# anzeA/Tarok

Measured on AMD Instinct MI355X. Metric: env steps/sec at 65 536 parallel 4-player games; 1/2/4/8 MI355X, higher is better.
Workload: dtype u64

## Files before the change

### tarok_amd/csrc/tarok_env.hip

```cpp
#include "tarok_device.h"

#include <hip/hip_runtime.h>
#include <stdint.h>
#include <stdio.h>
#include <stdlib.h>
#include <string.h>
#include <type_traits>
#include <utility>

#include "../../include/tarok_env.h"

#define TK_BLOCK 256
#define TK_PF_SLOTS (4 * TK_BLOCK)
#define TK_GRAPH_CACHE 16
#define TK_REFILL_CAP (TK_BLOCK * TK_AHEAD)
#define TK_REFILL_FAN 8
#define TK_RC(group, k) ((((size_t)(group)) * 4 + (k)) * 32)
#define TK_BULK_EVERY 32u
#define TK_BULK_CAP ((TK_BULK_EVERY / 4) * TK_BLOCK)

#define TK_AHEAD TAROK_GAMES_AHEAD
#define TK_LINE(episode) ((u32)(episode) % (u32)TK_AHEAD)
#define TK_FINQ 128
#define TK_STREAM_STORE(ptr, val) __builtin_nontemporal_store((val), (ptr))
// ... 53 lines not shown
#define HIPCHK(x)                                                   \
    do {                                                            \
        hipError_t e_ = (x);                                        \
        if (e_ != hipSuccess) { g_last_hip = (int)e_; return TAROK_EHIP; } \
    } while (0)

static inline dim3 grid_for(int64_t n) { return dim3((unsigned)((n + TK_BLOCK - 1) / TK_BLOCK)); }

__device__ __forceinline__ void load_game(Game &g, const ulonglong2 *s01, const ulonglong2 *s23, int64_t i) {
    ulonglong2 a = s01[i], b = s23[i];
    unpack(g, a.x, a.y, b.x, b.y);
}
__device__ __forceinline__ void store_game(const Game &g, ulonglong2 *s01, ulonglong2 *s23, int64_t i,
                                           bool seats_changed = true) {
    ulonglong2 a;
    pack_play(g, a.x, a.y);
    s01[i] = a;
    if (seats_changed) {
        ulonglong2 b;
        pack_seats(g, b.x, b.y);
        s23[i] = b;
    }
}

TK_KERNEL(TK_BLOCK, 80) void k_reset(
    int64_t n, u64 seed, u64 offset, u32 episode, int mix, int flags,
    const uint8_t *__restrict__ deals, const int8_t *__restrict__ contract, const int8_t *__restrict__ declarer,
    const int8_t *__restrict__ king, const int8_t *__restrict__ choice, const uint8_t *__restrict__ discards,
    ulonglong2 *__restrict__ s01, ulonglong2 *__restrict__ s23, Aux *aux, Counters *__restrict__ cnt,
    uint16_t *__restrict__ nstale, u64 *__restrict__ gkey) {
    TK_VGPR_TOP(80, 79);
    int64_t i = (int64_t)blockIdx.x * TK_BLOCK + threadIdx.x;
    if (i >= n) return;
    u64 key = game_key(seed, offset + (u64)i, episode);
    u64 h0 = 0, h1 = 0, h2 = 0, h3 = 0, tal = 0;
    bool bad = false;
#pragma unroll
    for (int b = 0; b < TK_AHEAD; b++) aux[i].line[b].nep = 0xFFFFFFFFu;
    nstale[i] = (uint16_t)((1u << TK_AHEAD) - 1);
    if (deals) {
        const uint8_t *p = deals + i * 54;
        u64 h[4] = {0, 0, 0, 0};
        u64 seen = 0;
        for (int k = 0; k < 48; k++) { u32 c = p[k]; bad |= c >= 54; c &= 63; seen |= 1ULL << c; h[k / 12] |= 1ULL << c; }
        for (int k = 0; k < 6; k++) { u32 c = p[48 + k]; bad |= c >= 54; c &= 63; seen |= 1ULL << c; tal |= (u64)c << (6 * k); }
        bad |= seen != TK_DECK;
        h0 = h[0]; h1 = h[1]; h2 = h[2]; h3 = h[3];
    } else {
        deal_thread(key, h0, h1, h2, h3, tal);
    }
    u32 c, d, k;
    if (contract) {
        int ci = contract[i];
        bad |= ci < 0 || ci > 9;
        c = (u32)ci % 10u;
        d = declarer ? ((u32)declarer[i] & 3u) : 0u;
        k = king ? ((u32)king[i] & 3u) : 0u;
    } else {
        sample_setup(key, mix, c, d, k);
    }
    Game g;
    setup_game(g, h0, h1, h2, h3, tal, c, d, k);
    g.epar = TK_LINE(episode); g.cprev = 0;
    if (g.phase == TK_PHASE_EXCHANGE && !(flags & TAROK_DEFER_EXCHANGE)) {
        if (choice && discards) {
            const uint8_t *q = discards + i * 3;
            apply_exchange(g, (u32)(uint8_t)choice[i], q[0], q[1], q[2]);
        } else {
            bot_exchange(g, key);
        }
    }
    if (bad) g.error = 1;
    store_game(g, s01, s23, i);
    gkey[i] = key;
    cnt[i].episode = episode;
    if (flags & TAROK_CLEAR_COUNTERS) cnt[i].score_sum = make_int4(0, 0, 0, 0);
}

__device__ __forceinline__ void deal_into_buffer(Aux *aux, int64_t j, u32 episode, u64 seed, u64 offset, int mix) {
    u64 key = game_key(seed, offset + (u64)j, (u64)episode);
    u64 h0, h1, h2, h3, tal;
    deal_thread(key, h0, h1, h2, h3, tal);
    u32 c, d, k;
    sample_setup(key, mix, c, d, k);
    Game g;
    setup_game(g, h0, h1, h2, h3, tal, c, d, k);
    g.epar = TK_LINE(episode); g.cprev = 0;
    if (g.phase == TK_PHASE_EXCHANGE) bot_exchange(g, key);
    ulonglong2 a, b;
    pack(g, a.x, a.y, b.x, b.y);
    AuxLine *ln = &aux[j].line[TK_LINE(episode)];
    ln->n01 = a; ln->n23 = b; ln->nkey = key; ln->nep = episode;
}

TK_KERNEL(TK_BLOCK, 128) void k_prefetch(int64_t n, u64 seed, u64 offset, int mix,
                                                      Aux *aux, const Counters *__restrict__ cnt,
                                                      uint16_t *__restrict__ nstale) {
    TK_VGPR_TOP(128, 127);
    __shared__ unsigned short list[TK_AHEAD * TK_PF_SLOTS];
    __shared__ u32 count;
    int64_t base = (int64_t)blockIdx.x * TK_PF_SLOTS;
    if (threadIdx.x == 0) count = 0;
    __syncthreads();
    const u64 ALL = (1u << TK_AHEAD) - 1;
    u64 f = reinterpret_cast<const u64 *>(nstale + base)[threadIdx.x];
    if (f) {
        u32 c = (u32)__popcll(f & (0x0001000100010001ULL * ALL));
        u32 pos = atomicAdd(&count, c);
#pragma unroll
        for (u32 k = 0; k < 4; k++) {
            u32 fk = (u32)(f >> (16 * k)) & (u32)ALL;
#pragma unroll
            for (u32 b = 0; b < TK_AHEAD; b++)
                if (fk & (1u << b)) list[pos++] = (unsigned short)((threadIdx.x * 4 + k) * TK_AHEAD + b);
        }
        reinterpret_cast<u64 *>(nstale + base)[threadIdx.x] = 0;
    }
    __syncthreads();
    u32 total = count;
    for (u32 j = threadIdx.x; j < total; j += TK_BLOCK) {
        int64_t i = base + list[j] / TK_AHEAD;
        if (i >= n) continue;
        deal_into_buffer(aux, i, cnt[i].episode + 1 + (list[j] % TK_AHEAD), seed, offset, mix);
    }
}

TK_KERNEL(TK_BLOCK, 64) void k_exchange(int64_t n, const int8_t *__restrict__ choice,
                                                      const uint8_t *__restrict__ discards,
                                                      ulonglong2 *__restrict__ s01, ulonglong2 *__restrict__ s23,
                                                      const u64 *__restrict__ gkey) {
    TK_VGPR_TOP(64, 63);
    int64_t i = (int64_t)blockIdx.x * TK_BLOCK + threadIdx.x;
    if (i >= n) return;
    Game g;
    load_game(g, s01, s23, i);
    if (g.phase != TK_PHASE_EXCHANGE) return;
    if (choice && discards) {
        const uint8_t *q = discards + i * 3;
        apply_exchange(g, (u32)(uint8_t)choice[i], q[0], q[1], q[2]);
    } else {
        bot_exchange(g, gkey[i]);
    }
    store_game(g, s01, s23, i);
}

TK_KERNEL(TK_BLOCK, 64) void k_legal(int64_t n, const ulonglong2 *__restrict__ s01,
                                                   const ulonglong2 *__restrict__ s23, u64 *__restrict__ obs,
                                                   int8_t *__restrict__ seat) {
    TK_VGPR_TOP(64, 63);
    int64_t i = (int64_t)blockIdx.x * TK_BLOCK + threadIdx.x;
    if (i >= n) return;
    Game g;
    load_game(g, s01, s23, i);
    obs[i] = obs_word(g, false);
    if (seat) seat[i] = (int8_t)((g.leader + g.nt) & 3);
}

TK_KERNEL(TK_BLOCK, 64) void k_policy(int64_t n, const u64 *__restrict__ obs,
                                                    const u64 *__restrict__ gkey, uint8_t *__restrict__ action) {
    TK_VGPR_TOP(64, 63);
    int64_t i = (int64_t)blockIdx.x * TK_BLOCK + threadIdx.x;
    if (i >= n) return;
    u64 o = obs[i], key = gkey[i];
    u64 m = o & TAROK_OBS_MASK;
    u32 a = 255;
    if (m) a = policy_action(key, (u32)(o >> TAROK_OBS_STEP_SHIFT) & 63u, m);
    action[i] = (uint8_t)a;
}

TK_KERNEL(TK_BLOCK, 64) void k_policy_x4(int64_t n, const u64 *__restrict__ obs,
                                                       const u64 *__restrict__ gkey, uint8_t *__restrict__ action) {
    TK_VGPR_TOP(64, 63);
    int64_t base = (int64_t)blockIdx.x * (4 * TK_BLOCK);
    if (base + 4 * TK_BLOCK <= n) {
        int64_t p0 = base + 2 * threadIdx.x, p1 = p0 + 2 * TK_BLOCK;
        ulonglong2 o0 = *reinterpret_cast<const ulonglong2 *>(obs + p0), o1 = *reinterpret_cast<const ulonglong2 *>(obs + p1);
        ulonglong2 k0 = *reinterpret_cast<const ulonglong2 *>(gkey + p0), k1 = *reinterpret_cast<const ulonglong2 *>(gkey + p1);
        auto one = [](u64 o, u64 key) __attribute__((always_inline)) {
            u64 m = o & TAROK_OBS_MASK;
            return m ? policy_action(key, (u32)(o >> TAROK_OBS_STEP_SHIFT) & 63u, m) : 255u;
        };
        u32 a0 = one(o0.x, k0.x) | (one(o0.y, k0.y) << 8), a1 = one(o1.x, k1.x) | (one(o1.y, k1.y) << 8);
        *reinterpret_cast<uint16_t *>(action + p0) = (uint16_t)a0;
        *reinterpret_cast<uint16_t *>(action + p1) = (uint16_t)a1;
        return;
    }
    for (int64_t i = base + threadIdx.x; i < n; i += TK_BLOCK) {
        u64 o = obs[i];
        u64 m = o & TAROK_OBS_MASK;
        u32 a = 255;
        if (m) a = policy_action(gkey[i], (u32)(o >> TAROK_OBS_STEP_SHIFT) & 63u, m);
        action[i] = (uint8_t)a;
    }
}

template <class T> __device__ __forceinline__ T tk_ld(const T *p) { return __hip_atomic_load(p, __ATOMIC_RELAXED, __HIP_MEMORY_SCOPE_AGENT); }

#define TK_EPOCH_SHARDS 256
#define TK_EPOCH_WORDS (32 * TK_EPOCH_SHARDS)
#define TK_PHASES (2u * TK_BULK_EVERY)
static_assert((TK_BULK_EVERY & (TK_BULK_EVERY - 1)) == 0 && TK_BULK_EVERY >= 4 && TK_BULK_EVERY + 1 <= 4 * (TK_AHEAD - 1),
              "a line is dealt at most TK_BULK_EVERY + 1 launches after it was emptied and is needed again TK_AHEAD - 1 games (four launches each, at least) after that");
struct TkCount { u32 own, other; };
__device__ __forceinline__ u32 tk_shard_size(u32 grid, u32 shard) { return (grid + TK_EPOCH_SHARDS - 1 - shard) / TK_EPOCH_SHARDS; }
template <int KIND> __device__ __forceinline__ u32 tk_other_grid(u32 groups, u32 fan) { return KIND == 0 ? groups + (groups + fan - 1) / fan : groups; }
template <int KIND> __device__ __forceinline__ u32 tk_other_shard(u32 groups) { return (KIND == 0 ? blockIdx.x : blockIdx.x % groups) % TK_EPOCH_SHARDS; }
template <int KIND> __device__ __forceinline__ TkCount launch_count(const u32 *epoch, u32 groups) {
    TkCount c;
    c.own = tk_ld(epoch + KIND * TK_EPOCH_WORDS + 32 * (blockIdx.x % TK_EPOCH_SHARDS));
    c.other = tk_ld(epoch + (1 - KIND) * TK_EPOCH_WORDS + 32 * tk_other_shard<KIND>(groups));
    return c;
}
__device__ __forceinline__ u32 tk_div_small(u32 count, u32 g) {
    u32 q = (u32)(((float)count + 0.5f) * __builtin_amdgcn_rcpf((float)g));
    q -= (q * g > count) ? 1u : 0u;
    q += ((q + 1u) * g <= count) ? 1u : 0u;
    return q;
}
template <int KIND> __device__ __forceinline__ u32 launch_phase(TkCount c, u32 groups, u32 fan) {
    asm volatile("" : "+v"(c.own), "+v"(c.other));
    u32 own = tk_div_small(c.own, tk_shard_size(gridDim.x, blockIdx.x % TK_EPOCH_SHARDS));
    u32 other = tk_div_small(c.other, tk_shard_size(tk_other_grid<KIND>(groups, fan), tk_other_shard<KIND>(groups)));
    return (own + other) % TK_PHASES;
}
template <int KIND> __device__ __forceinline__ void launch_counted(u32 *epoch) {
    if (threadIdx.x == 0)
        (void)atomicInc(epoch + KIND * TK_EPOCH_WORDS + 32 * (blockIdx.x % TK_EPOCH_SHARDS),
                        TK_PHASES * tk_shard_size(gridDim.x, blockIdx.x % TK_EPOCH_SHARDS) - 1u);
}

template <bool BULK>
__device__ __forceinline__ void refill_role(u32 rblock, u32 tid, u32 nthreads, u64 seed, u64 offset, int mix, u32 play_groups,
                                        TkCount count, u32 *epoch, u32 fan, bool bulk_on, Aux *aux, u64 *rlist, u32 *rcount, u64 *elist) {
    constexpr int KIND = BULK ? 0 : 1;
    const u32 kind_fan = fan;
    if (BULK) fan = 1;
    u32 g0 = rblock * fan;
    u32 len0[TK_REFILL_FAN], len1[TK_REFILL_FAN];
#pragma unroll
    for (u32 q = 0; q < TK_REFILL_FAN; q++) {
        bool has = q < fan && g0 + q < play_groups;
        len0[q] = has ? tk_ld(&rcount[TK_RC(g0 + q, 0)]) : 0u;
        len1[q] = has ? tk_ld(&rcount[TK_RC(g0 + q, 1)]) : 0u;
    }
    if (!BULK) {
        __syncthreads();
        launch_counted<KIND>(epoch);
    }
    const u32 phase = launch_phase<KIND>(count, play_groups, kind_fan), par = phase & 1u;
    if (!BULK) {
        if (tid < 2 * fan && g0 + tid / 2 < play_groups) rcount[TK_RC(g0 + tid / 2, 2 + (tid & 1))] = 0u;
    }
    u32 cum[TK_REFILL_FAN + 1];
    cum[0] = 0;
    u32 which = par ^ 1u;
    const u32 odd = 0u - par;
#pragma unroll
    for (u32 q = 0; q < TK_REFILL_FAN; q++) cum[q + 1] = cum[q] + ((len0[q] & odd) | (len1[q] & ~odd));
    const bool any = cum[TK_REFILL_FAN] != 0;
    u64 *lists = rlist;
    u32 cap = TK_REFILL_CAP;
    const bool bulk = BULK && bulk_on && phase % TK_BULK_EVERY == 0;
#pragma nounroll
    for (u32 pass = 0; pass < (BULK ? 2u : 1u); pass++) {
        if (pass == 1) {
            if (!bulk) break;
            which = ((phase / TK_BULK_EVERY) & 1u) ^ 1u;
            lists = elist; cap = TK_BULK_CAP;
#pragma unroll
            for (u32 q = 0; q < TK_REFILL_FAN; q++) {
                bool has = q < fan && g0 + q < play_groups;
                cum[q + 1] = cum[q] + (has ? min(tk_ld(&rcount[TK_RC(g0 + q, 2 + which)]), (u32)TK_BULK_CAP) : 0u);
            }
        }
        for (u32 j = tid; j < cum[TK_REFILL_FAN]; j += nthreads) {
            u32 q = 0;
#pragma unroll
            for (u32 r = 1; r < TK_REFILL_FAN; r++) q += j >= cum[r] ? 1u : 0u;
            u32 base = 0;
#pragma unroll
            for (u32 r = 0; r < TK_REFILL_FAN; r++) base = (r == q) ? cum[r] : base;
            u64 en = tk_ld(&lists[((int64_t)(g0 + q) * 2 + which) * cap + (j - base)]);
            deal_into_buffer(aux, (int64_t)(g0 + q) * TK_BLOCK + (u32)(en & 0xFFFF), (u32)(en >> 32), seed, offset, mix);
        }
    }
    if (any || bulk) {
        __syncthreads();
        if (any && tid < fan && g0 + tid < play_groups) rcount[TK_RC(g0 + tid, par ^ 1u)] = 0u;
        if (bulk && tid < fan && g0 + tid < play_groups) rcount[TK_RC(g0 + tid, 2 + which)] = 0u;
    }
}

template <bool HIST>
__device__ __forceinline__ void play_role(
    u32 group, u32 tid,
    int64_t n, u64 seed, u64 offset, int mix, int flags, int cards, int64_t stride, TkCount count, u32 *epoch, u32 play_groups, u32 fan,
    uint8_t *__restrict__ action_out, int16_t *__restrict__ reward,
    uint8_t *__restrict__ done, uint16_t *__restrict__ trick, u64 *__restrict__ obs, uint8_t *__restrict__ hist,
    ulonglong2 *__restrict__ s01, ulonglong2 *__restrict__ s23, Aux *aux, Counters *__restrict__ cnt,
    u64 *__restrict__ gkey, u64 *rlist, u32 *rcount, u64 *__restrict__ stamps) {
    __shared__ unsigned short push_list[TK_REFILL_CAP];
    __shared__ u32 push_ep[TK_BLOCK];
    __shared__ u32 push_count;
    __shared__ u32 finq[TK_BLOCK / 64][9][TK_FINQ];
    __shared__ int sacc[4][TK_BLOCK];
    if (tid == 0) push_count = 0;
    sacc[0][tid] = 0; sacc[1][tid] = 0; sacc[2][tid] = 0; sacc[3][tid] = 0;
    __syncthreads();
    u32 fq_head = 0, fq_n = 0;
    u32 (*fq)[TK_FINQ] = finq[tid >> 6];
    auto drain_finished = [&](u32 cnt_) __attribute__((always_inline)) {
        u32 lane = tid & 63;
        if (lane < cnt_) {
            u32 e = (fq_head + lane) & (TK_FINQ - 1);
            Game f;
            f.A = TK_U64(fq[0][e], fq[1][e]); f.B = TK_U64(fq[2][e], fq[3][e]); f.C = TK_U64(fq[4][e], fq[5][e]);
            u32 m = fq[7][e], ri = fq[8][e];
            f.talon = TK_U64(fq[6][e], (m >> 24) & 15u);
            f.contract = m & 15; f.declarer = (m >> 4) & 3; f.king = (m >> 6) & 3; f.team = (m >> 8) & 15;
            f.tl = (m >> 12) & 7; f.trick_no = (m >> 16) & 15; f.leader = (m >> 20) & 3;
            f.trick = 0; f.nt = 0; f.phase = TK_PHASE_DONE; f.error = 0; f.epar = 0; f.cprev = 0;
            u64 sc = final_scores(f);
            u32 t = ri & 0xFFFFu;
            if (reward) {
                u64 rs = sc;
                if ((flags & TAROK_REWARD_REF) && (f.contract == TK_BERAC || f.contract == TK_ODPRTI_BERAC)) {
                    int dv = f.trick_no >= 12 ? -20 : 20;
                    u32 d = f.declarer;
                    rs = pack_scores(d == 0 ? (int)(int16_t)(sc & 0xFFFF) : dv, d == 1 ? (int)(int16_t)((sc >> 16) & 0xFFFF) : dv,
                                     d == 2 ? (int)(int16_t)((sc >> 32) & 0xFFFF) : dv, d == 3 ? (int)(int16_t)(sc >> 48) : dv);
                }
                reinterpret_cast<u64 *>(reward)[(int64_t)group * TK_BLOCK + t + (int64_t)(ri >> 16) * stride] = rs;
            }
            atomicAdd(&sacc[0][t], (int)(int16_t)(sc & 0xFFFF)); atomicAdd(&sacc[1][t], (int)(int16_t)((sc >> 16) & 0xFFFF));
            atomicAdd(&sacc[2][t], (int)(int16_t)((sc >> 32) & 0xFFFF)); atomicAdd(&sacc[3][t], (int)(int16_t)(sc >> 48));
        }
        fq_head = (fq_head + cnt_) & (TK_FINQ - 1);
        fq_n -= cnt_;
    };
    u64 t_real0 = 0, t_cyc0 = 0, t_play = 0;
    if (stamps) { t_real0 = __builtin_amdgcn_s_memrealtime(); t_cyc0 = __builtin_amdgcn_s_memtime(); }
    int64_t i = (int64_t)group * TK_BLOCK + tid;
    bool valid = i < n;
    int64_t ic = valid ? i : n - 1;
    Game g;
    load_game(g, s01, s23, ic);
    u64 key = gkey[ic];
    bool autoreset = (flags & TAROK_AUTO_RESET) != 0;
    bool berac = g.contract == TK_BERAC || g.contract == TK_ODPRTI_BERAC;
    bool spec = valid && ((g.phase == TK_PHASE_PLAY && (int)g.nt + cards >= 4 &&
                           (berac || (int)(g.trick_no * 4 + g.nt) + cards >= 48)) ||
                          g.phase == TK_PHASE_DONE);
    u32 cprev0 = valid ? g.cprev : 0u;
    u32 allowed = TK_AHEAD - min(cprev0, (u32)TK_AHEAD);
    int4 acc = make_int4(0, 0, 0, 0);
    u32 cur_ep = 0;
    ulonglong2 na = make_ulonglong2(0, 0), nb = na, na2 = na, nb2 = na;
    u64 nkey = 0, nkey2 = 0;
    u32 nep1 = 0, nep2 = 0;
    bool ok1 = false, ok2 = false;
    auto line_tag = [&](bool &ok, u32 &nep, u32 tag) __attribute__((always_inline)) { nep = tag; ok = true; };
    if (spec) {
        acc = cnt[i].score_sum;
        cur_ep = cnt[i].episode;
        if (autoreset && allowed > 0) {
            const AuxLine *ln = &aux[i].line[TK_LINE(g.epar + 1)];
            na = ln->n01; nb = ln->n23; nkey = ln->nkey;
            line_tag(ok1, nep1, ln->nep);
            if (allowed > 1 && cards > 4) {
                const AuxLine *l2 = &aux[i].line[TK_LINE(g.epar + 2)];
                na2 = l2->n01; nb2 = l2->n23; nkey2 = l2->nkey;
                line_tag(ok2, nep2, l2->nep);
            }
        }
    }
    TK_WAIT_LOADS();
    u32 par = launch_phase<1>(count, play_groups, fan) & 1u;
    launch_counted<1>(epoch);
    g.cprev = 0;
    u32 consumed = 0;
    bool resync = false;
    bool blocked = false;
    bool acc_dirty = false, seats_dirty = false, touched = false;
    u64 legal = (valid && g.phase == TK_PHASE_PLAY) ? legal_now(g) : 0;
    u64 c_lead = 0;
    u64 pending = 0;
    u32 blocked_v = 0, resync_v = 0;
    auto fetch_lines = [&](bool lacks, bool lacks2) __attribute__((always_inline)) {
        if (lacks) {
            const AuxLine *ln = &aux[i].line[TK_LINE(cur_ep + 1)];
            na = ln->n01; nb = ln->n23; nkey = ln->nkey;
            line_tag(ok1, nep1, ln->nep);
        }
        if (lacks2) {
            const AuxLine *l2 = &aux[i].line[TK_LINE(cur_ep + 2)];
            na2 = l2->n01; nb2 = l2->n23; nkey2 = l2->nkey;
            line_tag(ok2, nep2, l2->nep);
        }
    };
    auto play_card = [&](auto all_tag, auto nt_tag, auto std_tag, int64_t row, int ci) __attribute__((always_inline)) {
        constexpr bool ALL = decltype(all_tag)::value;
        constexpr int NT = decltype(nt_tag)::value;
        constexpr bool STD = decltype(std_tag)::value;
        if constexpr (NT >= 0) g.nt = (u32)NT;
        constexpr bool TOP_UP_EARLY = ALL && NT == 0;
        constexpr bool TOP_UP_LATE = !(ALL && NT == 3);
        if constexpr (TOP_UP_EARLY) {
            if (TK_RARE(pending != 0)) {
                pending = 0;
                bool base = spec && blocked_v == 0 && consumed >= 1;
                bool lacks = base && nep1 != cur_ep + 1 && consumed < allowed;
                bool lacks2 = base && nep2 != cur_ep + 2 && consumed + 1 < allowed;
                fetch_lines(lacks, lacks2);
            }
        }
        const bool v = ALL ? true : valid;
        const bool play = ALL ? true : (valid && g.phase == TK_PHASE_PLAY);
        u32 a = play ? policy_action(key, g.trick_no * 4 + g.nt, legal) : 255u;
        u64 scores = 0;
        u32 trick_info = 0;
        int res = -2;
        const u32 pos = g.trick_no * 4 + g.nt;
        if constexpr (ALL && NT == 0) c_lead = g.C;
        const u64 *lead_plane = (ALL && NT >= 0) ? &c_lead : nullptr;
        if (play) res = apply_step<true, true>(g, a, scores, trick_info, !STD && trick != nullptr, lead_plane);
        bool fin = res == 1;
        if (HIST && hist && play && res >= 0) hist[(int64_t)pos * n + i] = (uint8_t)a;
        if constexpr (!(ALL && NT >= 0)) {
            touched = touched || res != -2;
            seats_dirty = seats_dirty || (res >= 0 && g.nt == 0);
        }
        if (v) {
            if (STD || action_out) TK_STREAM_STORE(&action_out[row], (uint8_t)a);
            if (!STD && trick) TK_STREAM_STORE(&trick[row], (uint16_t)trick_info);
        }
        constexpr bool CAN_END = !(ALL && NT >= 0 && NT < 3);
        constexpr bool FAST_RENEW = ALL && NT == 3;
        auto push_finished = [&](u64 fm, u32 slot0) __attribute__((always_inline)) {
            u32 e = (slot0 + __builtin_amdgcn_mbcnt_hi((u32)(fm >> 32), __builtin_amdgcn_mbcnt_lo((u32)fm, 0))) & (TK_FINQ - 1);
            fq[0][e] = TK_LO(g.A); fq[1][e] = TK_HI(g.A); fq[2][e] = TK_LO(g.B); fq[3][e] = TK_HI(g.B);
            fq[4][e] = TK_LO(g.C); fq[5][e] = TK_HI(g.C); fq[6][e] = TK_LO(g.talon);
            u32 m = (g.declarer << 4) | g.contract;      TK_KEEP_VGPR(m);
            m = (g.king << 6) | m;                       TK_KEEP_VGPR(m);
            m = (g.team << 8) | m;                       TK_KEEP_VGPR(m);
            m = (g.tl << 12) | m;                        TK_KEEP_VGPR(m);
            m = (g.trick_no << 16) | m;                  TK_KEEP_VGPR(m);
            m = (g.leader << 20) | m;                    TK_KEEP_VGPR(m);
            fq[7][e] = (TK_HI(g.talon) << 24) | m;
            fq[8][e] = ((u32)ci << 16) | tid;
        };
        auto swap_in = [&]() __attribute__((always_inline)) {
            unpack_fresh(g, na.x, na.y, nb.x, nb.y);
            key = nkey;
            na = na2; nb = nb2; nkey = nkey2;
            nep1 = nep2;
        };
        auto deal_in_place = [&](bool deal_here, Game &gd, u64 &kd) __attribute__((always_inline)) {
            u64 pend = __ballot(deal_here);
            if (TK_RARE(pend != 0)) {
                u64 dkey = 0;
                if (deal_here) dkey = game_key(seed, offset + (u64)i, cur_ep + 1);
                u64 h0 = 0, h1 = 0, h2 = 0, h3 = 0, tal = 0;
                u32 lane = __lane_id();
                while (pend) {
                    int l = __builtin_ctzll(pend);
                    pend &= pend - 1;
                    u32 klo = (u32)__builtin_amdgcn_readlane((int)(u32)dkey, l);
                    u32 khi = (u32)__builtin_amdgcn_readlane((int)(u32)(dkey >> 32), l);
                    u64 w0, w1, w2, w3, wt;
                    deal_wave(klo, khi, w0, w1, w2, w3, wt);
                    if (lane == (u32)l) { h0 = w0; h1 = w1; h2 = w2; h3 = w3; tal = wt; }
                }
                if (deal_here) {
                    u32 cc, d, k;
                    sample_setup(dkey, mix, cc, d, k);
                    setup_game(gd, h0, h1, h2, h3, tal, cc, d, k);
                    gd.epar = TK_LINE(cur_ep + 1); gd.cprev = 0;
                    if (gd.phase == TK_PHASE_EXCHANGE) bot_exchange(gd, dkey);
                    kd = dkey;
                }
            }
        };
        if constexpr (FAST_RENEW) {
            u64 fm = __ballot(fin);
            if (TK_USUAL(fm != 0)) {
                if (TK_RARE(fq_n >= 64)) drain_finished(64);
                const u32 slot0 = fq_head + fq_n;
                fq_n += (u32)__popcll(fm);
                if (TK_RARE((fm & __ballot(nep1 != cur_ep + 1)) != 0)) {
                    bool lineless = fin && nep1 != cur_ep + 1;
                    resync_v |= (lineless && consumed < allowed) ? 1u : 0u;
                    blocked_v |= lineless ? 1u : 0u;
                    Game d = g;
                    u64 dk = key;
                    deal_in_place(lineless, d, dk);
                    if (lineless) { pack(d, na.x, na.y, nb.x, nb.y); nkey = dk; nep1 = cur_ep + 1; }
                }
                pending |= fm & __ballot(nep2 != cur_ep + 2);
                if (fin) { push_finished(fm, slot0); swap_in(); cur_ep++; consumed++; }
            }
        }
        if constexpr (CAN_END && !FAST_RENEW) {
            u64 fm = __ballot(fin);
            if (TK_USUAL(fm != 0)) {
                if (TK_RARE(fq_n >= 64)) drain_finished(64);
                if (fin) push_finished(fm, fq_head + fq_n);
                fq_n += (u32)__popcll(fm);
            }
        }
        if (CAN_END && !FAST_RENEW && (ALL || autoreset)) {
            bool renew = ALL ? fin : (v && g.phase == TK_PHASE_DONE);
            if (TK_USUAL(__ballot(renew) != 0)) {
                if constexpr (TOP_UP_LATE) {
                    bool lacks = spec && !blocked && !ok1 && consumed >= 1 && consumed < allowed;
                    if (TK_RARE(__ballot(renew && lacks) != 0)) {
                        bool lacks2 = spec && !blocked && !ok2 && consumed >= 1 && consumed + 1 < allowed;
                        fetch_lines(lacks, lacks2);
                        TK_WAIT_LOADS();
                    }
                }
                bool swap = renew && !blocked && ok1 && nep1 == cur_ep + 1;
                if (swap) {
                    swap_in();
                    ok1 = ok2 && consumed + 1 < allowed;
                    ok2 = false;
                }
                bool deal_here = renew && !swap;
                if (deal_here && consumed < allowed) resync = true;
                if (deal_here) blocked = true;
                deal_in_place(deal_here, g, key);
                if (renew) { cur_ep++; consumed++; seats_dirty = true; }
            }
        }
        legal = (ALL || (v && g.phase == TK_PHASE_PLAY)) ? legal_now(g) : 0;
        if (v) {
            const u32 fin01 = ALL ? (u32)res : (fin ? 1u : 0u);
            TK_STREAM_STORE(&obs[row], obs_word_with<true>(g, false, legal) | ((u64)(ALL ? fin01 : ((fin || g.phase == TK_PHASE_DONE) ? 1u : 0u)) << 62));
            if (STD || done) TK_STREAM_STORE(&done[row], (uint8_t)fin01);
        }
    };
    int64_t row = i;
    typedef std::integral_constant<int, -1> nt_any;
    if (autoreset && __ballot(valid && g.phase == TK_PHASE_PLAY) == ~0ULL) {
        if ((cards & 3) == 0 && __ballot(g.nt != 0) == 0) {
            auto tricks = [&](auto std_tag) __attribute__((always_inline)) {
                touched = true; seats_dirty = true;
                for (int c = 0; c < cards; c += 4) {
                    play_card(std::true_type{}, std::integral_constant<int, 0>{}, std_tag, row, c); row += stride;
                    play_card(std::true_type{}, std::integral_constant<int, 1>{}, std_tag, row, c + 1); row += stride;
                    play_card(std::true_type{}, std::integral_constant<int, 2>{}, std_tag, row, c + 2); row += stride;
                    play_card(std::true_type{}, std::integral_constant<int, 3>{}, std_tag, row, c + 3); row += stride;
                }
            };
            if (action_out && done && !trick) tricks(std::true_type{});
            else tricks(std::false_type{});
        } else {
            for (int c = 0; c < cards; c++, row += stride) play_card(std::true_type{}, nt_any{}, std::false_type{}, row, c);
        }
    } else {
        for (int c = 0; c < cards; c++, row += stride) play_card(std::false_type{}, nt_any{}, std::false_type{}, row, c);
    }
    while (fq_n) drain_finished(min(fq_n, 64u));
    __builtin_amdgcn_s_waitcnt(0xC07F);
    {
        int4 sa = make_int4(sacc[0][tid], sacc[1][tid], sacc[2][tid], sacc[3][tid]);
        if (sa.x | sa.y | sa.z | sa.w) { acc.x += sa.x; acc.y += sa.y; acc.z += sa.z; acc.w += sa.w; acc_dirty = true; }
    }
    u32 np = (resync || resync_v != 0) ? (u32)TK_AHEAD : min(consumed, (u32)TK_AHEAD);
    if (valid) {
        g.cprev = np;
        if (acc_dirty) cnt[i].score_sum = acc;
        if (consumed) { cnt[i].episode = cur_ep; gkey[i] = key; }
        if (touched || consumed || cprev0 != np) store_game(g, s01, s23, i, seats_dirty || cprev0 != np);
    }
    if (stamps) t_play = __builtin_amdgcn_s_memtime() - t_cyc0;
    if (valid && np) {
        u32 pos = atomicAdd(&push_count, np);
        push_ep[tid] = cur_ep;
        for (u32 j = 0; j < np; j++) push_list[pos + j] = (unsigned short)(j * TK_BLOCK + tid);
    }
    __syncthreads();
    u32 total = push_count;
    u64 *lst = rlist + ((int64_t)group * 2 + par) * TK_REFILL_CAP;
    for (u32 j = tid; j < total; j += TK_BLOCK) {
        u32 en = push_list[j], t = en % TK_BLOCK;
        lst[j] = ((u64)(push_ep[t] + TK_AHEAD - en / TK_BLOCK) << 32) | t;
    }
    if (tid == 0) rcount[TK_RC(group, par)] = total;
    if (stamps && (tid & 63) == 0) {
        u64 w = (u64)i >> 6;
        stamps[3 * w + 0] = t_real0;
        stamps[3 * w + 1] = __builtin_amdgcn_s_memrealtime();
        stamps[3 * w + 2] = ((__builtin_amdgcn_s_memtime() - t_cyc0) << 32) | (t_play & 0xFFFFFFFFULL);
    }
}

#define TK_PLAY_ARGS                                                                                                             \
    int64_t n, u64 seed, u64 offset, int mix, int flags, int cards, int64_t stride, u32 play_groups, u32 *epoch, u32 fan,         \
        uint8_t *__restrict__ action_out, int16_t *__restrict__ reward,                                                           \
        uint8_t *__restrict__ done, uint16_t *__restrict__ trick, u64 *__restrict__ obs, uint8_t *__restrict__ hist,              \
        ulonglong2 *__restrict__ s01, ulonglong2 *__restrict__ s23, Aux *aux, Counters *__restrict__ cnt,                         \
        u64 *__restrict__ gkey, u64 *rlist, u32 *rcount, u64 *__restrict__ stamps
template <bool HIST>
TK_KERNEL(TK_BLOCK, 168) __attribute__((amdgpu_waves_per_eu(3, 3))) void k_play_wide(TK_PLAY_ARGS) {
    TK_VGPR_TOP(168, 167);
    TkCount count = launch_count<1>(epoch, play_groups);
    if (blockIdx.x >= play_groups)
        refill_role<false>(blockIdx.x - play_groups, threadIdx.x, TK_BLOCK, seed, offset, mix, play_groups, count, epoch, fan, false, aux, rlist, rcount, nullptr);
    else {
        play_role<HIST>(blockIdx.x, threadIdx.x, n, seed, offset, mix, flags, cards, stride, count, epoch, play_groups, fan,
                        action_out, reward, done, trick, obs, hist, s01, s23, aux, cnt, gkey, rlist, rcount, stamps);
    }
}

__device__ __forceinline__ void deal_in_place_wave(bool deal_here, Game &gd, u64 &kd, u64 seed, u64 offset, int64_t i, u32 ep, int mix) {
    u64 pend = __ballot(deal_here);
    if (pend == 0) return;
    u64 dkey = 0;
    if (deal_here) dkey = game_key(seed, offset + (u64)i, ep);
    u64 h0 = 0, h1 = 0, h2 = 0, h3 = 0, tal = 0;
    u32 lane = __lane_id();
    while (pend) {
        int l = __builtin_ctzll(pend);
        pend &= pend - 1;
        u32 klo = (u32)__builtin_amdgcn_readlane((int)(u32)dkey, l);
        u32 khi = (u32)__builtin_amdgcn_readlane((int)(u32)(dkey >> 32), l);
        u64 w0, w1, w2, w3, wt;
        deal_wave(klo, khi, w0, w1, w2, w3, wt);
        if (lane == (u32)l) { h0 = w0; h1 = w1; h2 = w2; h3 = w3; tal = wt; }
    }
    if (deal_here) {
        u32 cc, d, k;
        sample_setup(dkey, mix, cc, d, k);
        setup_game(gd, h0, h1, h2, h3, tal, cc, d, k);
        gd.epar = TK_LINE(ep); gd.cprev = 0;
        if (gd.phase == TK_PHASE_EXCHANGE) bot_exchange(gd, dkey);
        kd = dkey;
    }
}

#define FINQ_WORDS 13
template <bool RANDOM, bool LAZY>
__device__ __forceinline__ void step_role(
    u32 group, u32 tid, bool active, u32 a_reg, bool lazy_on,
    int64_t n, u64 seed, u64 offset, int mix, int flags, TkCount count, u32 *epoch, u32 play_groups, u32 fan,
    const uint8_t *__restrict__ action_in, uint8_t *__restrict__ action_out, int16_t *__restrict__ reward,
    uint8_t *__restrict__ done, uint16_t *__restrict__ trick, u64 *__restrict__ obs, uint8_t *__restrict__ hist,
    ulonglong2 *__restrict__ s01, ulonglong2 *__restrict__ s23, Aux *aux, Counters *__restrict__ cnt,
    u64 *__restrict__ gkey, u64 *rlist, u32 *rcount, u64 *elist,
    u32 (*__restrict__ finq)[TK_BLOCK] ) {
    __shared__ unsigned short push_list[TK_REFILL_CAP];
    __shared__ u32 push_ep[TK_BLOCK];
    __shared__ u32 push_count, fin_count, late_count;
    __shared__ u64 late_list[LAZY ? TK_BLOCK : 1];
    const bool lazy = LAZY && lazy_on;
    if (tid == 0) { push_count = 0; fin_count = 0; late_count = 0; }
    u32 efill0 = 0, efill1 = 0;
    if (lazy) { efill0 = tk_ld(&rcount[TK_RC(group, 2)]); efill1 = tk_ld(&rcount[TK_RC(group, 3)]); }
    __syncthreads();
    int64_t i = (int64_t)group * TK_BLOCK + tid;
    bool valid = active && i < n;
    int64_t ic = valid ? i : n - 1;
    Game g;
    load_game(g, s01, s23, ic);
    u64 key = 0;
    u32 a = 255;
    if (RANDOM) key = gkey[ic]; else a = action_in ? action_in[ic] : a_reg;
    const bool autoreset = (flags & TAROK_AUTO_RESET) != 0;
    const u32 cprev0 = valid ? g.cprev : 0u;
    const u32 allowed = TK_AHEAD - min(cprev0, (u32)TK_AHEAD);
    int4 acc = make_int4(0, 0, 0, 0);
    u32 cur_ep = 0;
    ulonglong2 na = make_ulonglong2(0, 0), nb = na;
    u64 nkey = 0;
    u32 ntag = 0;
    bool have_line = false;
    auto load_finish = [&](bool need) __attribute__((always_inline)) {
        if (need) {
            acc = cnt[i].score_sum;
            cur_ep = cnt[i].episode;
            if (autoreset && allowed > 0) {
                const AuxLine *ln = &aux[i].line[TK_LINE(g.epar + 1)];
                na = ln->n01; nb = ln->n23; nkey = ln->nkey; ntag = ln->nep;
                have_line = true;
            }
        }
    };
    launch_counted<LAZY ? 0 : 1>(epoch);
    g.cprev = 0;
    const bool play = valid && g.phase == TK_PHASE_PLAY;
    const u32 pos = g.trick_no * 4 + g.nt;
    if (RANDOM) a = play ? policy_action(key, pos, legal_now(g)) : 255u;
    u64 scores = 0;
    u32 trick_info = 0;
    int res = -2;
    if (play) res = apply_step<RANDOM, true>(g, a, scores, trick_info, trick != nullptr, nullptr);
    const bool fin = res == 1;
    if (hist && play && res >= 0) hist[(int64_t)pos * n + i] = (uint8_t)a;
    bool seats_dirty = res >= 0 && g.nt == 0;
    if (valid) {
        if (RANDOM && action_out) TK_STREAM_STORE(&action_out[i], (uint8_t)a);
        if (trick) TK_STREAM_STORE(&trick[i], (uint16_t)trick_info);
    }
    const bool renew = autoreset && valid && g.phase == TK_PHASE_DONE;
    load_finish(fin || renew);
    if (fin) {
        u32 e = atomicAdd(&fin_count, 1u);
        finq[0][e] = TK_LO(g.A); finq[1][e] = TK_HI(g.A); finq[2][e] = TK_LO(g.B); finq[3][e] = TK_HI(g.B);
        finq[4][e] = TK_LO(g.C); finq[5][e] = TK_HI(g.C); finq[6][e] = TK_LO(g.talon);
        finq[7][e] = g.contract | (g.declarer << 4) | (g.king << 6) | (g.team << 8) | (g.tl << 12) | (g.trick_no << 16) | (g.leader << 20) |
                     (TK_HI(g.talon) << 24);
        finq[8][e] = tid;
        finq[9][e] = (u32)acc.x; finq[10][e] = (u32)acc.y; finq[11][e] = (u32)acc.z; finq[12][e] = (u32)acc.w;
    }
    u32 consumed = 0;
    bool resync = false;
    if (__ballot(renew) != 0) {
        bool swap = renew && have_line && ntag == cur_ep + 1;
        if (swap) { unpack_fresh(g, na.x, na.y, nb.x, nb.y); key = nkey; }
        bool deal_here = renew && !swap;
        resync = deal_here && allowed > 0;
        deal_in_place_wave(deal_here, g, key, seed, offset, i, cur_ep + 1, mix);
        if (renew) { cur_ep++; consumed = 1; seats_dirty = true; }
    }
    if (valid) {
        TK_STREAM_STORE(&obs[i], obs_word(g, fin));
        if (done) TK_STREAM_STORE(&done[i], (uint8_t)(fin ? 1 : 0));
    }
    const u32 np = resync ? (u32)TK_AHEAD : (lazy ? 0u : consumed);
    if (valid) {
        g.cprev = np;
        if (consumed) { cnt[i].episode = cur_ep; gkey[i] = key; }
        if (res != -2 || consumed || cprev0 != np) store_game(g, s01, s23, i, seats_dirty || cprev0 != np);
    }
    if (valid && np) {
        u32 p0 = atomicAdd(&push_count, np);
        push_ep[tid] = cur_ep;
        for (u32 j = 0; j < np; j++) push_list[p0 + j] = (unsigned short)(j * TK_BLOCK + tid);
    }
    if (lazy && valid && consumed && !resync) late_list[atomicAdd(&late_count, 1u)] = ((u64)(cur_ep + TK_AHEAD) << 32) | tid;
    __syncthreads();
    if (active)
        for (u32 e = tid, nf = fin_count; e < nf; e += TK_BLOCK) {
            Game f;
            f.A = TK_U64(finq[0][e], finq[1][e]); f.B = TK_U64(finq[2][e], finq[3][e]); f.C = TK_U64(finq[4][e], finq[5][e]);
            u32 m = finq[7][e], t = finq[8][e];
            f.talon = TK_U64(finq[6][e], (m >> 24) & 15u);
            f.contract = m & 15; f.declarer = (m >> 4) & 3; f.king = (m >> 6) & 3; f.team = (m >> 8) & 15;
            f.tl = (m >> 12) & 7; f.trick_no = (m >> 16) & 15; f.leader = (m >> 20) & 3;
            f.trick = 0; f.nt = 0; f.phase = TK_PHASE_DONE; f.error = 0; f.epar = 0; f.cprev = 0;
            u64 sc = final_scores(f);
            int64_t it = (int64_t)group * TK_BLOCK + t;
            if (reward) {
                u64 rs = sc;
                if ((flags & TAROK_REWARD_REF) && (f.contract == TK_BERAC || f.contract == TK_ODPRTI_BERAC)) {
                    int dv = f.trick_no >= 12 ? -20 : 20;
                    u32 d = f.declarer;
                    rs = pack_scores(d == 0 ? (int)(int16_t)(sc & 0xFFFF) : dv, d == 1 ? (int)(int16_t)((sc >> 16) & 0xFFFF) : dv,
                                     d == 2 ? (int)(int16_t)((sc >> 32) & 0xFFFF) : dv, d == 3 ? (int)(int16_t)(sc >> 48) : dv);
                }
                reinterpret_cast<u64 *>(reward)[it] = rs;
            }
            cnt[it].score_sum = make_int4((int)finq[9][e] + (int16_t)(sc & 0xFFFF), (int)finq[10][e] + (int16_t)((sc >> 16) & 0xFFFF),
                                          (int)finq[11][e] + (int16_t)((sc >> 32) & 0xFFFF), (int)finq[12][e] + (int16_t)(sc >> 48));
        }
    const u32 total = push_count, late = lazy ? late_count : 0u;
    if ((total | late) == 0) return;
    const u32 phase = launch_phase<LAZY ? 0 : 1>(count, play_groups, fan), par = phase & 1u;
    if (total) {
        u64 *lst = rlist + ((int64_t)group * 2 + par) * TK_REFILL_CAP;
        if (active)
            for (u32 j = tid; j < total; j += TK_BLOCK) {
                u32 en = push_list[j], t = en % TK_BLOCK;
                lst[j] = ((u64)(push_ep[t] + TK_AHEAD - en / TK_BLOCK) << 32) | t;
            }
        if (tid == 0) rcount[TK_RC(group, par)] = total;
    }
    if (lazy && late) {
        const u32 eb = (phase / TK_BULK_EVERY) & 1u;
        const u32 fill = eb ? efill1 : efill0;
        u64 *el = elist + ((int64_t)group * 2 + eb) * TK_BULK_CAP;
        if (active && tid < late && fill + tid < TK_BULK_CAP) el[fill + tid] = late_list[tid];
        if (tid == 0) rcount[TK_RC(group, 2 + eb)] = min(fill + late, (u32)TK_BULK_CAP);
    }
}

#define TK_STEP_ARGS                                                                                                              \
    int64_t n, u64 seed, u64 offset, int mix, int flags, u32 play_groups, u32 *epoch, u32 fan,                                    \
        const uint8_t *__restrict__ action_in, uint8_t *__restrict__ action_out, int16_t *__restrict__ reward,                    \
        uint8_t *__restrict__ done, uint16_t *__restrict__ trick, u64 *__restrict__ obs, uint8_t *__restrict__ hist,              \
        ulonglong2 *__restrict__ s01, ulonglong2 *__restrict__ s23, Aux *aux, Counters *__restrict__ cnt,                         \
        u64 *__restrict__ gkey, u64 *rlist, u32 *rcount, u64 *elist
template <bool RANDOM, bool LAZY>
TK_KERNEL(TK_BLOCK, 128) __attribute__((amdgpu_waves_per_eu(4))) void k_step(TK_STEP_ARGS) {
    TK_VGPR_TOP(128, 127);
    TkCount count = launch_count<LAZY ? 0 : 1>(epoch, play_groups);
    __shared__ u32 finq[FINQ_WORDS][TK_BLOCK];
    if (LAZY) {
        step_role<RANDOM, true>(blockIdx.x, threadIdx.x, true, 255u, true, n, seed, offset, mix, flags, count, epoch, play_groups, fan, action_in,
                                action_out, reward, done, trick, obs, hist, s01, s23, aux, cnt, gkey, rlist, rcount, elist, finq);
        refill_role<true>(blockIdx.x, threadIdx.x, TK_BLOCK, seed, offset, mix, play_groups, count, epoch, fan, true, aux, rlist, rcount, elist);
    } else {
        u32 q = blockIdx.x / (fan + 1), r = blockIdx.x % (fan + 1);
        if (r == 0)
            refill_role<false>(q, threadIdx.x, TK_BLOCK, seed, offset, mix, play_groups, count, epoch, fan, false, aux, rlist, rcount, elist);
        else
            step_role<RANDOM, false>(blockIdx.x - q - 1, threadIdx.x, true, 255u, false, n, seed, offset, mix, flags, count, epoch, play_groups, fan,
                                     action_in, action_out, reward, done, trick, obs, hist, s01, s23, aux, cnt, gkey, rlist, rcount, elist, finq);
    }
}

TK_KERNEL(TK_BLOCK, 96) void k_rollout(int64_t n, u64 seed, u64 offset, u32 episode, int mix,
                                                     int16_t *__restrict__ scores_out, int16_t *__restrict__ nsteps_out,
                                                     int8_t *__restrict__ seats, u64 *__restrict__ masks,
                                                     uint8_t *__restrict__ actions) {
    TK_VGPR_TOP(96, 95);
    int64_t i = (int64_t)blockIdx.x * TK_BLOCK + threadIdx.x;
    if (i >= n) return;
    u64 key = game_key(seed, offset + (u64)i, episode);
    u64 h0, h1, h2, h3, tal;
    deal_thread(key, h0, h1, h2, h3, tal);
    u32 c, d, k;
    sample_setup(key, mix, c, d, k);
    Game g;
    setup_game(g, h0, h1, h2, h3, tal, c, d, k);
    if (g.phase == TK_PHASE_EXCHANGE) bot_exchange(g, key);
    u64 scores = 0;
    int played = 0;
    auto card = [&](auto nt_tag, int t) __attribute__((always_inline)) {
        constexpr int NT = decltype(nt_tag)::value;
        bool live = g.phase == TK_PHASE_PLAY;
        u64 m = 0;
        u32 a = 255;
        int seat = -1;
        if (live) {
            g.nt = (u32)NT;
            m = legal_now(g);
            seat = (int)((g.leader + g.nt) & 3);
            a = policy_action(key, (u32)t, m);
            u32 ti;
            apply_step<true>(g, a, scores, ti);
            played++;
        }
        if (seats) seats[(int64_t)t * n + i] = (int8_t)seat;
        if (masks) masks[(int64_t)t * n + i] = m;
        if (actions) actions[(int64_t)t * n + i] = (uint8_t)a;
    };
    for (int t = 0; t < 48; t += 4) {
        card(std::integral_constant<int, 0>{}, t);
        card(std::integral_constant<int, 1>{}, t + 1);
        card(std::integral_constant<int, 2>{}, t + 2);
        card(std::integral_constant<int, 3>{}, t + 3);
    }
    if (scores_out) reinterpret_cast<u64 *>(scores_out)[i] = scores;
    if (nsteps_out) nsteps_out[i] = (int16_t)played;
}

__device__ __forceinline__ void policy_feature_words(const Game &g, u64 (&e)[4]) {
    u32 seat = (g.leader + g.nt) & 3;
    bool live = g.phase == TK_PHASE_PLAY;
    u64 on_table = 0;
    for (u32 j = 0; j < g.nt; j++) on_table |= 1ULL << ((g.trick >> (6 * j)) & 63);
    u64 f1 = (u64)(1u << ((g.declarer - seat) & 3)) | ((u64)(1u << g.nt) << 4) | ((u64)((g.team >> seat) & 1) << 8) |
// ... 1702 lines not shown
```

Measured before the change: 186.9 billion.

## Stage prefetched episode lines in LDS double buffer and vectorize finish-queue LDS stores

The prefetched next-episode deal lines (two 128-bit halves plus key, for two episodes ahead) move out of per-thread registers into a parity-indexed shared-memory double buffer. Loads issued by the early top-up at trick position 0 are written to LDS later, at position 2, so their latency is hidden. The finished-game queue is repacked from nine scalar u32 arrays into two uint4 arrays plus one u32 array, so pushes and drains use 128-bit LDS accesses. The aim is to cut VGPR pressure and LDS instruction count, in exchange for roughly 20 KB more LDS per block, which could limit occupancy, and extra LDS round trips on every episode swap.

```diff
diff --git a/tarok_amd/csrc/tarok_env.hip b/tarok_amd/csrc/tarok_env.hip
--- a/tarok_amd/csrc/tarok_env.hip
+++ b/tarok_amd/csrc/tarok_env.hip
@@ -379,21 +379,26 @@
     __shared__ unsigned short push_list[TK_REFILL_CAP];
     __shared__ u32 push_ep[TK_BLOCK];
     __shared__ u32 push_count;
-    __shared__ u32 finq[TK_BLOCK / 64][9][TK_FINQ];
+    __shared__ __attribute__((aligned(16))) uint4 finq_ab[TK_BLOCK / 64][TK_FINQ], finq_cm[TK_BLOCK / 64][TK_FINQ];
+    __shared__ u32 finq_ri[TK_BLOCK / 64][TK_FINQ];
+    __shared__ ulonglong2 line01[2][TK_BLOCK], line23[2][TK_BLOCK];
+    __shared__ u64 linekey[2][TK_BLOCK];
     __shared__ int sacc[4][TK_BLOCK];
     if (tid == 0) push_count = 0;
     sacc[0][tid] = 0; sacc[1][tid] = 0; sacc[2][tid] = 0; sacc[3][tid] = 0;
     __syncthreads();
     u32 fq_head = 0, fq_n = 0;
-    u32 (*fq)[TK_FINQ] = finq[tid >> 6];
+    uint4 *fq_ab = finq_ab[tid >> 6], *fq_cm = finq_cm[tid >> 6];
+    u32 *fq_ri = finq_ri[tid >> 6];
     auto drain_finished = [&](u32 cnt_) __attribute__((always_inline)) {
         u32 lane = tid & 63;
         if (lane < cnt_) {
             u32 e = (fq_head + lane) & (TK_FINQ - 1);
             Game f;
-            f.A = TK_U64(fq[0][e], fq[1][e]); f.B = TK_U64(fq[2][e], fq[3][e]); f.C = TK_U64(fq[4][e], fq[5][e]);
-            u32 m = fq[7][e], ri = fq[8][e];
-            f.talon = TK_U64(fq[6][e], (m >> 24) & 15u);
+            const uint4 ab = fq_ab[e], cm = fq_cm[e];
+            f.A = TK_U64(ab.x, ab.y); f.B = TK_U64(ab.z, ab.w); f.C = TK_U64(cm.x, cm.y);
+            u32 m = cm.w, ri = fq_ri[e];
+            f.talon = TK_U64(cm.z, (m >> 24) & 15u);
             f.contract = m & 15; f.declarer = (m >> 4) & 3; f.king = (m >> 6) & 3; f.team = (m >> 8) & 15;
             f.tl = (m >> 12) & 7; f.trick_no = (m >> 16) & 15; f.leader = (m >> 20) & 3;
             f.trick = 0; f.nt = 0; f.phase = TK_PHASE_DONE; f.error = 0; f.epar = 0; f.cprev = 0;
@@ -432,26 +437,48 @@
     u32 allowed = TK_AHEAD - min(cprev0, (u32)TK_AHEAD);
     int4 acc = make_int4(0, 0, 0, 0);
     u32 cur_ep = 0;
-    ulonglong2 na = make_ulonglong2(0, 0), nb = na, na2 = na, nb2 = na;
-    u64 nkey = 0, nkey2 = 0;
+    struct LineLoad {
+        u64 a0, a1, b0, b1, k, c0, c1, d0, d1, k2;
+        u32 which;
+        bool any;
+    };
     u32 nep1 = 0, nep2 = 0;
     bool ok1 = false, ok2 = false;
     auto line_tag = [&](bool &ok, u32 &nep, u32 tag) __attribute__((always_inline)) { nep = tag; ok = true; };
-    if (spec) {
-        acc = cnt[i].score_sum;
-        cur_ep = cnt[i].episode;
-        if (autoreset && allowed > 0) {
-            const AuxLine *ln = &aux[i].line[TK_LINE(g.epar + 1)];
-            na = ln->n01; nb = ln->n23; nkey = ln->nkey;
-            line_tag(ok1, nep1, ln->nep);
-            if (allowed > 1 && cards > 4) {
-                const AuxLine *l2 = &aux[i].line[TK_LINE(g.epar + 2)];
-                na2 = l2->n01; nb2 = l2->n23; nkey2 = l2->nkey;
-                line_tag(ok2, nep2, l2->nep);
+    auto put_line = [&](u32 ep, u64 a0, u64 a1, u64 b0, u64 b1, u64 k) __attribute__((always_inline)) {
+        const u32 p = ep & 1u;
+        line01[p][tid] = make_ulonglong2(a0, a1); line23[p][tid] = make_ulonglong2(b0, b1); linekey[p][tid] = k;
+    };
+    auto put_lines = [&](const LineLoad &ll) __attribute__((always_inline)) {
+        if (ll.which & 1u) put_line(cur_ep + 1, ll.a0, ll.a1, ll.b0, ll.b1, ll.k);
+        if (ll.which & 2u) put_line(cur_ep + 2, ll.c0, ll.c1, ll.d0, ll.d1, ll.k2);
+    };
+    auto get_line = [&](const AuxLine *ln, u64 &a0, u64 &a1, u64 &b0, u64 &b1, u64 &k) __attribute__((always_inline)) {
+        const ulonglong2 a = ln->n01, b = ln->n23;
+        a0 = a.x; a1 = a.y; b0 = b.x; b1 = b.y; k = ln->nkey;
+    };
+    {
+        LineLoad ll;
+        ll.which = 0;
+        if (spec) {
+            acc = cnt[i].score_sum;
+            cur_ep = cnt[i].episode;
+            if (autoreset && allowed > 0) {
+                const AuxLine *ln = &aux[i].line[TK_LINE(g.epar + 1)];
+                get_line(ln, ll.a0, ll.a1, ll.b0, ll.b1, ll.k);
+                line_tag(ok1, nep1, ln->nep);
+                ll.which = 1;
+                if (allowed > 1 && cards > 4) {
+                    const AuxLine *l2 = &aux[i].line[TK_LINE(g.epar + 2)];
+                    get_line(l2, ll.c0, ll.c1, ll.d0, ll.d1, ll.k2);
+                    line_tag(ok2, nep2, l2->nep);
+                    ll.which = 3;
+                }
             }
         }
-    }
-    TK_WAIT_LOADS();
+        TK_WAIT_LOADS();
+        put_lines(ll);
+    }
     u32 par = launch_phase<1>(count, play_groups, fan) & 1u;
     launch_counted<1>(epoch);
     g.cprev = 0;
@@ -463,19 +490,20 @@
     u64 c_lead = 0;
     u64 pending = 0;
     u32 blocked_v = 0, resync_v = 0;
-    auto fetch_lines = [&](bool lacks, bool lacks2) __attribute__((always_inline)) {
+    auto fetch_lines = [&](bool lacks, bool lacks2, LineLoad &ll) __attribute__((always_inline)) {
+        ll.which = (lacks ? 1u : 0u) | (lacks2 ? 2u : 0u);
         if (lacks) {
             const AuxLine *ln = &aux[i].line[TK_LINE(cur_ep + 1)];
-            na = ln->n01; nb = ln->n23; nkey = ln->nkey;
+            get_line(ln, ll.a0, ll.a1, ll.b0, ll.b1, ll.k);
             line_tag(ok1, nep1, ln->nep);
         }
         if (lacks2) {
             const AuxLine *l2 = &aux[i].line[TK_LINE(cur_ep + 2)];
-            na2 = l2->n01; nb2 = l2->n23; nkey2 = l2->nkey;
+            get_line(l2, ll.c0, ll.c1, ll.d0, ll.d1, ll.k2);
             line_tag(ok2, nep2, l2->nep);
         }
     };
-    auto play_card = [&](auto all_tag, auto nt_tag, auto std_tag, int64_t row, int ci) __attribute__((always_inline)) {
+    auto play_card = [&](auto all_tag, auto nt_tag, auto std_tag, int64_t row, int ci, LineLoad &ll) __attribute__((always_inline)) {
         constexpr bool ALL = decltype(all_tag)::value;
         constexpr int NT = decltype(nt_tag)::value;
         constexpr bool STD = decltype(std_tag)::value;
@@ -488,8 +516,12 @@
                 bool base = spec && blocked_v == 0 && consumed >= 1;
                 bool lacks = base && nep1 != cur_ep + 1 && consumed < allowed;
                 bool lacks2 = base && nep2 != cur_ep + 2 && consumed + 1 < allowed;
-                fetch_lines(lacks, lacks2);
+                fetch_lines(lacks, lacks2, ll);
+                ll.any = true;
             }
+        }
+        if constexpr (ALL && NT == 2) {
+            if (TK_RARE(ll.any)) put_lines(ll);
         }
         const bool v = ALL ? true : valid;
         const bool play = ALL ? true : (valid && g.phase == TK_PHASE_PLAY);
@@ -515,21 +547,21 @@
         constexpr bool FAST_RENEW = ALL && NT == 3;
         auto push_finished = [&](u64 fm, u32 slot0) __attribute__((always_inline)) {
             u32 e = (slot0 + __builtin_amdgcn_mbcnt_hi((u32)(fm >> 32), __builtin_amdgcn_mbcnt_lo((u32)fm, 0))) & (TK_FINQ - 1);
-            fq[0][e] = TK_LO(g.A); fq[1][e] = TK_HI(g.A); fq[2][e] = TK_LO(g.B); fq[3][e] = TK_HI(g.B);
-            fq[4][e] = TK_LO(g.C); fq[5][e] = TK_HI(g.C); fq[6][e] = TK_LO(g.talon);
+            fq_ab[e] = make_uint4(TK_LO(g.A), TK_HI(g.A), TK_LO(g.B), TK_HI(g.B));
             u32 m = (g.declarer << 4) | g.contract;      TK_KEEP_VGPR(m);
             m = (g.king << 6) | m;                       TK_KEEP_VGPR(m);
             m = (g.team << 8) | m;                       TK_KEEP_VGPR(m);
             m = (g.tl << 12) | m;                        TK_KEEP_VGPR(m);
             m = (g.trick_no << 16) | m;                  TK_KEEP_VGPR(m);
             m = (g.leader << 20) | m;                    TK_KEEP_VGPR(m);
-            fq[7][e] = (TK_HI(g.talon) << 24) | m;
-            fq[8][e] = ((u32)ci << 16) | tid;
+            fq_cm[e] = make_uint4(TK_LO(g.C), TK_HI(g.C), TK_LO(g.talon), (TK_HI(g.talon) << 24) | m);
+            fq_ri[e] = ((u32)ci << 16) | tid;
         };
         auto swap_in = [&]() __attribute__((always_inline)) {
-            unpack_fresh(g, na.x, na.y, nb.x, nb.y);
-            key = nkey;
-            na = na2; nb = nb2; nkey = nkey2;
+            const u32 p = (cur_ep + 1) & 1u;
+            const ulonglong2 a = line01[p][tid], b = line23[p][tid];
+            key = linekey[p][tid];
+            unpack_fresh(g, a.x, a.y, b.x, b.y);
             nep1 = nep2;
         };
         auto deal_in_place = [&](bool deal_here, Game &gd, u64 &kd) __attribute__((always_inline)) {
@@ -571,10 +603,24 @@
                     Game d = g;
                     u64 dk = key;
                     deal_in_place(lineless, d, dk);
-                    if (lineless) { pack(d, na.x, na.y, nb.x, nb.y); nkey = dk; nep1 = cur_ep + 1; }
+                    if (lineless) {
+                        u64 a0, a1, b0, b1;
+                        pack(d, a0, a1, b0, b1);
+                        put_line(cur_ep + 1, a0, a1, b0, b1, dk);
+                        nep1 = cur_ep + 1;
+                    }
                 }
                 pending |= fm & __ballot(nep2 != cur_ep + 2);
-                if (fin) { push_finished(fm, slot0); swap_in(); cur_ep++; consumed++; }
+                if (fin) {
+                    const u32 p = (cur_ep + 1) & 1u;
+                    const ulonglong2 a = line01[p][tid], b = line23[p][tid];
+                    const u64 k = linekey[p][tid];
+                    push_finished(fm, slot0);
+                    unpack_fresh(g, a.x, a.y, b.x, b.y);
+                    key = k;
+                    nep1 = nep2;
+                    cur_ep++; consumed++;
+                }
             }
         }
         if constexpr (CAN_END && !FAST_RENEW) {
@@ -592,8 +638,9 @@
                     bool lacks = spec && !blocked && !ok1 && consumed >= 1 && consumed < allowed;
                     if (TK_RARE(__ballot(renew && lacks) != 0)) {
                         bool lacks2 = spec && !blocked && !ok2 && consumed >= 1 && consumed + 1 < allowed;
-                        fetch_lines(lacks, lacks2);
+                        fetch_lines(lacks, lacks2, ll);
                         TK_WAIT_LOADS();
+                        put_lines(ll);
                     }
                 }
                 bool swap = renew && !blocked && ok1 && nep1 == cur_ep + 1;
@@ -623,19 +670,21 @@
             auto tricks = [&](auto std_tag) __attribute__((always_inline)) {
                 touched = true; seats_dirty = true;
                 for (int c = 0; c < cards; c += 4) {
-                    play_card(std::true_type{}, std::integral_constant<int, 0>{}, std_tag, row, c); row += stride;
-                    play_card(std::true_type{}, std::integral_constant<int, 1>{}, std_tag, row, c + 1); row += stride;
-                    play_card(std::true_type{}, std::integral_constant<int, 2>{}, std_tag, row, c + 2); row += stride;
-                    play_card(std::true_type{}, std::integral_constant<int, 3>{}, std_tag, row, c + 3); row += stride;
+                    LineLoad ll;
+                    ll.any = false;
+                    play_card(std::true_type{}, std::integral_constant<int, 0>{}, std_tag, row, c, ll); row += stride;
+                    play_card(std::true_type{}, std::integral_constant<int, 1>{}, std_tag, row, c + 1, ll); row += stride;
+                    play_card(std::true_type{}, std::integral_constant<int, 2>{}, std_tag, row, c + 2, ll); row += stride;
+                    play_card(std::true_type{}, std::integral_constant<int, 3>{}, std_tag, row, c + 3, ll); row += stride;
                 }
             };
             if (action_out && done && !trick) tricks(std::true_type{});
             else tricks(std::false_type{});
         } else {
-            for (int c = 0; c < cards; c++, row += stride) play_card(std::true_type{}, nt_any{}, std::false_type{}, row, c);
+            for (int c = 0; c < cards; c++, row += stride) { LineLoad ll; play_card(std::true_type{}, nt_any{}, std::false_type{}, row, c, ll); }
         }
     } else {
-        for (int c = 0; c < cards; c++, row += stride) play_card(std::false_type{}, nt_any{}, std::false_type{}, row, c);
+        for (int c = 0; c < cards; c++, row += stride) { LineLoad ll; play_card(std::false_type{}, nt_any{}, std::false_type{}, row, c, ll); }
     }
     while (fq_n) drain_finished(min(fq_n, 64u));
     __builtin_amdgcn_s_waitcnt(0xC07F);
```

Result: slower. 183.2 billion (-2.0%).
